# tataganesh/Query-Efficient-Approx-to-improve-OCR

Measured on AMD Instinct MI355X. Metric: patch-images/sec UNet->CRNN->CTC fwd+bwd, 32x128 grey, higher is better.
Workload: dtype f32 (GEMMs as scaled 2 x fp16 split products — three fp16 MFMAs per fp32 multiply-add — fp32 accumulate); 1 GPU; BASELINE configs[2]: full minibatch step of train_nn_area.py:212-287 — Phase A (UNet eval fwd, TopKCER k = 5 % of the minibatch, inner_limit = 4 jitter replicas fused in the batch dim, CRNN train-BN fwd+bwd, Adam(CRNN)) + Phase B (UNet train-BN -> CRNN BN-eval -> CTC mean + MSE -> backward -> Adam(UNet)) + greedy decode -> CER -> update_cer (:290-304) on synthetic POS-style 32x128 patches; batch_per_gpu=2048, global_batch=2048, full_step=True, crnn_wgrad=True, parallelism=dp1, hipgraph=False

## Files before the change

query-efficient-approx-to-improve-ocr_amd/csrc/conv_halo16.hip:

```cpp
#include "conv_args.h"
#include <type_traits>

using qea_conv::ConvArgs;

namespace {

__device__ const float qea_zero16[4] = {0.f, 0.f, 0.f, 0.f};

constexpr int halo_m16_wgs(int cout) { return cout == 32 ? 3 : 2; }

template <int COUT, bool STATS, int IMW = 0, int PKW = 0, bool BST = false>
__global__ __launch_bounds__(256) __attribute__((amdgpu_waves_per_eu(halo_m16_wgs(COUT), halo_m16_wgs(COUT)))) void conv3x3_halo_m16_kernel(
    const float* __restrict__ x, const _Float16* __restrict__ wf, float* __restrict__ y, int B, int H, int W, int ldx, int ldy,
    const float* __restrict__ scale, const float* __restrict__ bias, int relu, double* __restrict__ stats, int chunks, int Ntot,
    const float* __restrict__ mask, int ldmask, int total, const float* __restrict__ xmax, float* __restrict__ yamax, float* __restrict__ pooled,
    int ldp, float* __restrict__ pamax, const float* __restrict__ yref, int ldyref, const double* __restrict__ bst64, const float* __restrict__ bsc,
    const float* __restrict__ bsh) {
  constexpr int CIN = 64, TH = 4;
  constexpr bool SMALL = IMW != 0;
  constexpr int IMH = SMALL ? IMW / 4 : 1;
  constexpr int IPX = SMALL ? 32 / IMW : 1, IPY = SMALL ? TH / IMH : 1;
  constexpr int TW = 32, HW_ = SMALL ? IPX * (IMW + 2) : TW + 2, HH = SMALL ? TH + 1 : TH + 2, HP = HH * HW_;
  static_assert(!SMALL || COUT == 128, "small-image tiles: one wave row");
  constexpr int WN = COUT / 32, WM = 4 / WN, MI = TH / WM;
// ... 313 lines not shown
      }
      if (relu) {
#pragma unroll
        for (int i = 0; i < MI; ++i)
#pragma unroll
          for (int t = 0; t < 4; ++t)
#pragma unroll
            for (int r = 0; r < 4; ++r) acc[i][t][r] = fmaxf(acc[i][t][r], 0.f);
      }
      auto store_rows = [&](auto has_mask) {
        constexpr bool HAS_MASK = decltype(has_mask)::value;
#pragma unroll
        for (int i = 0; i < MI; ++i) {
          const int rowpix = (cur.b * H + cur.y0 + wm * MI + i) * W + cur.x0;
          float* yb = y + (size_t)rowpix * ldy;
          const float* mb = HAS_MASK ? mask + (size_t)rowpix * ldmask : nullptr;
          const int lo = 4 * lg * ldy + nbase, lom = 4 * lg * ldmask + nbase;
#pragma unroll
          for (int e = 0; e < 16; ++e) {
            const int g2 = (e >> 2) & 1;
            const int c = (e >> 3) * 16 + (e & 3);
            float v = acc[i][e >> 2][e & 3];
            if (SMALL) {
              const int px = c + 4 * lg;
              const int img = (i / IMH) * IPX + px / IMW;
              const size_t prow = ((size_t)(cur.b + img) * IMH + i % IMH) * IMW + px % IMW;
              if (cur.b + img >= B) continue;
              const int n = nbase + g2 * 16;
              if (HAS_MASK) v = (mask[prow * ldmask + n] > 0.f) ? v : 0.f;
              y[prow * ldy + n] = v;
            } else {
              if (HAS_MASK) v = (mb[lom + c * ldmask + g2 * 16] > 0.f) ? v : 0.f;
              yb[lo + c * ldy + g2 * 16] = v;
            }
            am = qea_amax_acc(am, v);
            if (STATS) {
              st0[g2] += (double)v;
              st1[g2] += (double)v * (double)v;
            }
          }
        }
      };
      if (mask) store_rows(std::true_type{});
      else store_rows(std::false_type{});
    }
    if (STATS || BST) {
#pragma unroll
      for (int g2 = 0; g2 < 2; ++g2) {
        double sa = st0[g2], sc = st1[g2];
        sa += __shfl_xor(sa, 16, 64);
        sc += __shfl_xor(sc, 16, 64);
        sa += __shfl_xor(sa, 32, 64);
        sc += __shfl_xor(sc, 32, 64);
        if (lg == 0) {
          double* dst = stats + ((size_t)(cur.tile_id * WM + wm) * Ntot + nbase + g2 * 16) * 2;
          dst[0] = sa;
          dst[1] = sc;
        }
      }
    }
    if (!has_next) break;
    cur = nxt;
    vb = nvb;
  }
  qea_amax_commit_block(am, yamax);
  if constexpr (PKW != 0) qea_amax_commit_block(pm, pamax);
}

template <int COUT, bool STATS, int IMW = 0, int PKW = 0, bool BST = false>
int launch_halo_m16_(const ConvArgs& a, hipStream_t s) {
  constexpr size_t lds = IMW ? (size_t)2 * (4 + 1) * (32 / IMW) * (IMW + 2) * 64 * 2 : (size_t)2 * (4 + 2) * 34 * 64 * 2;
  auto kern = conv3x3_halo_m16_kernel<COUT, STATS, IMW, PKW, BST>;
  static int attr_rc = (int)hipFuncSetAttribute((const void*)kern, hipFuncAttributeMaxDynamicSharedMemorySize, (int)lds);
  if (attr_rc != (int)hipSuccess) {
    qea_set_error("qea_conv_igemm(halo m16): cannot reserve %zu bytes of LDS: %s", (size_t)lds, hipGetErrorString((hipError_t)attr_rc));
    return QEA_ERR_LAUNCH;
  }
  const long long total = IMW ? (long long)qea_cdiv(a.B, (32 / IMW) * (4 / (IMW / 4))) * (a.N / COUT) : (long long)a.B * (a.H / 4) * (a.W / 32) * (a.N / COUT);
  if (total <= 0 || total > 0x7fffffffLL) {
    qea_set_error("qea_conv_igemm(halo m16): grid %lld out of range", total);
    return QEA_ERR_INVALID;
  }
  static const int resident = [] {
    int dev = 0, cus = 256;
    (void)hipGetDevice(&dev);
    (void)hipDeviceGetAttribute(&cus, hipDeviceAttributeMultiprocessorCount, dev);
    return halo_m16_wgs(COUT) * (cus & ~7);
  }();
  const unsigned grid = (total > resident && COUT > 32) ? (unsigned)resident : (unsigned)total;
  hipLaunchKernelGGL(kern, dim3(grid), dim3(256), lds, s, a.x, (const _Float16*)a.wp, a.y, a.B, a.H, a.W, a.ldx, a.ldy, a.scale, a.bias, a.relu, a.stats,
                     a.Cin / 64, a.N, a.mask, a.ldmask, (int)total, a.xmax, a.yamax, a.pool_y, a.ldpool, a.pool_amax, a.bst_y, a.ldbst, a.bst64, a.bst_scale,
                     a.bst_shift);
  return QEA_OK;
}

template <int COUT, int IMW = 0>
int launch_halo_m16(const ConvArgs& a, hipStream_t s) {
  if (a.pool_y) {
    if constexpr (COUT != 32 && IMW != 8) {
      if (a.pool_kw == 1) {
        if constexpr (COUT == 128 && IMW == 0) return launch_halo_m16_<COUT, false, IMW, 1>(a, s);
      } else {
        return launch_halo_m16_<COUT, false, IMW, 2>(a, s);
      }
    }
    qea_set_error("qea_conv_igemm(halo m16): no fused-pool instance for this shape");
    return QEA_ERR_INVALID;
  }
  if (a.bst_y) return launch_halo_m16_<COUT, false, IMW, 0, true>(a, s);
  return a.stats ? launch_halo_m16_<COUT, true, IMW>(a, s) : launch_halo_m16_<COUT, false, IMW>(a, s);
}

}

namespace qea_conv {

int launch_halo_m16_any(int n_sel, int sm, const ConvArgs& a, hipStream_t s) {
  if (sm == 16) return launch_halo_m16<128, 16>(a, s);
  if (sm == 8) return launch_halo_m16<128, 8>(a, s);
  if (n_sel == 32) return launch_halo_m16<32>(a, s);
  if (n_sel == 64) return launch_halo_m16<64>(a, s);
  return launch_halo_m16<128>(a, s);
}

}
```

query-efficient-approx-to-improve-ocr_amd/csrc/conv_igemm.hip:

```cpp
#include "conv_args.h"
#include <type_traits>
#include <stdlib.h>
#include <string.h>

using qea_conv::ConvArgs;
using qea_conv::conv_epilogue;

namespace {

template <int A_LD, int B_LD, int BK, int RPP>
struct IgemmGather {
  int lrow, kc, ntaps;
  int a_pix[A_LD];
  int a_ih0[A_LD], a_iw0[A_LD];
  const float* b_ptr[B_LD > 0 ? B_LD : 1];
  f32x4 a_reg[A_LD], b_reg[B_LD > 0 ? B_LD : 1];

  __device__ __forceinline__ void init(const ConvArgs& p, int tid, int m0, int n0) {
    constexpr int KCH = BK / 4;
    lrow = tid / KCH;
    kc = tid % KCH;
    ntaps = p.KH * p.KW;
    const int ohw = p.OH * p.OW;
#pragma unroll
// ... 1226 lines not shown
              st1 += (double)v * (double)v;
            }
          }
        }
      };
      if (mask) store_rows(std::true_type{});
      else store_rows(std::false_type{});
    }
    if (STATS || BST) {
      const double sa = st0 + __shfl_xor(st0, 32, 64);
      const double sc = st1 + __shfl_xor(st1, 32, 64);
      if (fh == 0) {
        double* dst = stats + ((size_t)(cur.tile_id * WM + wm) * Ntot + n) * 2;
        dst[0] = sa;
        dst[1] = sc;
      }
    }
    if (!has_next) break;
    cur = nxt;
    vb = nvb;
  }
  qea_amax_commit_block(am, yamax);
  if constexpr (PKW != 0) qea_amax_commit_block(pm, pamax);
}

__global__ void pack_frag_planes_kernel(const float* __restrict__ w, __bf16* __restrict__ dst, int N, int Cin, int CW) {
  const int NB = N > 128 ? 128 : N;
  const int KSr = CW / 16, WNr = NB / 32, chunks = Cin / CW;
  const int i = blockIdx.x * blockDim.x + threadIdx.x;
  if (i >= (N / NB) * chunks * 9 * KSr * WNr * 64) return;
  const int lane = i & 63;
  const int nj = (i >> 6) % WNr;
  const int gst = (i >> 6) / WNr;
  const int nbk = gst / (chunks * 9 * KSr);
  const int chunk = (gst / (9 * KSr)) % chunks, st = gst % (9 * KSr);
  const int tap = st / KSr, cs = st % KSr;
  const int n = nbk * NB + nj * 32 + (lane & 31);
  const float* src = w + ((size_t)n * 9 + tap) * Cin + chunk * CW + cs * 16 + 8 * (lane >> 5);
  const f32x4 v0 = *reinterpret_cast<const f32x4*>(src), v1 = *reinterpret_cast<const f32x4*>(src + 4);
  bf16x4 h0, m0, l0, h1, m1, l1;
  qea_split3(v0, h0, m0, l0);
  qea_split3(v1, h1, m1, l1);
  bf16x8 pl[3];
#pragma unroll
  for (int k = 0; k < 4; ++k) {
    pl[0][k] = h0[k]; pl[0][k + 4] = h1[k];
    pl[1][k] = m0[k]; pl[1][k + 4] = m1[k];
    pl[2][k] = l0[k]; pl[2][k + 4] = l1[k];
  }
#pragma unroll
  for (int p = 0; p < 3; ++p) *reinterpret_cast<bf16x8*>(dst + ((((size_t)gst * 3 + p) * WNr + nj) * 64 + lane) * 8) = pl[p];
}

__global__ void pack_frag_planes_f16_kernel(const float* __restrict__ w, _Float16* __restrict__ dst, int N, int Cin, int CW,
                                            const float* __restrict__ wmax) {
  const int NB = N > 128 ? 128 : N;
  const int KSr = CW / 16, WNr = NB / 32, chunks = Cin / CW;
  float sw, inv;
  qea_f16_scale(wmax[0], sw, inv);
  const int i = blockIdx.x * blockDim.x + threadIdx.x;
  if (i == 0) reinterpret_cast<float*>(dst + (size_t)N * 9 * Cin * 2)[0] = inv;
  if (i >= (N / NB) * chunks * 9 * KSr * WNr * 64) return;
  const int lane = i & 63;
  const int nj = (i >> 6) % WNr;
  const int gst = (i >> 6) / WNr;
  const int nbk = gst / (chunks * 9 * KSr);
  const int chunk = (gst / (9 * KSr)) % chunks, st = gst % (9 * KSr);
  const int tap = st / KSr, cs = st % KSr;
  const int n = nbk * NB + nj * 32 + (lane & 31);
  const float* src = w + ((size_t)n * 9 + tap) * Cin + chunk * CW + cs * 16 + 8 * (lane >> 5);
  const f32x4 v0 = *reinterpret_cast<const f32x4*>(src), v1 = *reinterpret_cast<const f32x4*>(src + 4);
  f16x4 h0, l0, h1, l1;
  qea_split2_f16(v0, sw, h0, l0);
  qea_split2_f16(v1, sw, h1, l1);
  f16x8 pl[2];
#pragma unroll
  for (int k = 0; k < 4; ++k) {
    pl[0][k] = h0[k]; pl[0][k + 4] = h1[k];
    pl[1][k] = l0[k]; pl[1][k + 4] = l1[k];
  }
#pragma unroll
  for (int p = 0; p < 2; ++p) *reinterpret_cast<f16x8*>(dst + ((((size_t)gst * 2 + p) * WNr + nj) * 64 + lane) * 8) = pl[p];
}

__global__ void pack_frag_planes_f16_m16_kernel(const float* __restrict__ w, _Float16* __restrict__ dst, int N, int Cin, const float* __restrict__ wmax) {
  const int NB = N > 128 ? 128 : N;
  const int NGr = NB / 16, chunks = Cin / 64;
  float sw, inv;
  qea_f16_scale(wmax[0], sw, inv);
  const int i = blockIdx.x * blockDim.x + threadIdx.x;
  if (i == 0) reinterpret_cast<float*>(dst + (size_t)N * 9 * Cin * 2)[0] = inv;
  if (i >= (N / NB) * chunks * 18 * NGr * 64) return;
  const int lane = i & 63;
  const int ng = (i >> 6) % NGr;
  const int gst = (i >> 6) / NGr;
  const int nbk = gst / (chunks * 18);
  const int chunk = (gst / 18) % chunks, st = gst % 18;
  const int tap = st / 2, ks = st % 2;
  const int n = nbk * NB + ng * 16 + (lane & 15);
  const float* src = w + ((size_t)n * 9 + tap) * Cin + chunk * 64 + ks * 32 + 8 * (lane >> 4);
  const f32x4 v0 = *reinterpret_cast<const f32x4*>(src), v1 = *reinterpret_cast<const f32x4*>(src + 4);
  f16x4 h0, l0, h1, l1;
  qea_split2_f16(v0, sw, h0, l0);
  qea_split2_f16(v1, sw, h1, l1);
  f16x8 pl[2];
#pragma unroll
  for (int k = 0; k < 4; ++k) {
    pl[0][k] = h0[k]; pl[0][k + 4] = h1[k];
    pl[1][k] = l0[k]; pl[1][k + 4] = l1[k];
  }
#pragma unroll
  for (int p = 0; p < 2; ++p) *reinterpret_cast<f16x8*>(dst + ((((size_t)gst * 2 + p) * NGr + ng) * 64 + lane) * 8) = pl[p];
}

template <int CIN, int COUT, int TH, bool STATS, int IMW = 0, int NPL = 3, int PKW = 0, bool BST = false>
int launch_halo_bf3_(const ConvArgs& a, hipStream_t s) {
  constexpr size_t lds = IMW ? (size_t)NPL * (TH + 1) * (32 / IMW) * (IMW + 2) * CIN * 2 : (size_t)NPL * (TH + 2) * 34 * CIN * 2;
  auto kern = conv3x3_halo_bf3_kernel<CIN, COUT, TH, STATS, IMW, NPL, PKW, BST>;
  static int attr_rc = (int)hipFuncSetAttribute((const void*)kern, hipFuncAttributeMaxDynamicSharedMemorySize, (int)lds);
  if (attr_rc != (int)hipSuccess) {
    qea_set_error("qea_conv_igemm(halo bf3): cannot reserve %zu bytes of LDS: %s", (size_t)lds, hipGetErrorString((hipError_t)attr_rc));
    return QEA_ERR_LAUNCH;
  }
  const long long total = IMW ? (long long)qea_cdiv(a.B, (32 / IMW) * (TH / (IMW / 4))) * (a.N / COUT)
                              : (long long)a.B * (a.H / TH) * (a.W / 32) * (a.N / COUT);
  if (total <= 0 || total > 0x7fffffffLL) {
    qea_set_error("qea_conv_igemm(halo bf3): grid %lld out of range", total);
    return QEA_ERR_INVALID;
  }
  static const int resident = [] {
    int dev = 0, cus = 256;
    (void)hipGetDevice(&dev);
    (void)hipDeviceGetAttribute(&cus, hipDeviceAttributeMultiprocessorCount, dev);
    return halo_bf3_wgs(CIN, COUT, NPL, BST) * (cus & ~7);
  }();
  const unsigned grid = (total > resident && COUT > 32) ? (unsigned)resident : (unsigned)total;
  hipLaunchKernelGGL(kern, dim3(grid), dim3(256), lds, s, a.x, (const __bf16*)a.wp, a.y, a.B, a.H, a.W, a.ldx, a.ldy,
                     a.scale, a.bias, a.relu, a.stats, a.Cin / CIN, a.N, a.mask, a.ldmask, (int)total, a.xmax, a.yamax, a.pool_y, a.ldpool, a.pool_amax,
                     a.bst_y, a.ldbst, a.bst64, a.bst_scale, a.bst_shift);
  return QEA_OK;
}

template <int CIN, int COUT, int TH, int IMW = 0>
int launch_halo_bf3_pool(const ConvArgs& a, hipStream_t s) {
  if (a.pool_kw == 1) return launch_halo_bf3_<CIN, COUT, TH, false, IMW, 2, 1>(a, s);
  return launch_halo_bf3_<CIN, COUT, TH, false, IMW, 2, 2>(a, s);
}

template <int CIN, int COUT, int TH, int IMW = 0>
int launch_halo_bf3(const ConvArgs& a, hipStream_t s) {
  if (a.xmax && a.bst_y)
    return launch_halo_bf3_<CIN, COUT, TH, false, IMW, 2, 0, true>(a, s);
  if (a.xmax)
    return a.stats ? launch_halo_bf3_<CIN, COUT, TH, true, IMW, 2>(a, s) : launch_halo_bf3_<CIN, COUT, TH, false, IMW, 2>(a, s);
  return a.stats ? launch_halo_bf3_<CIN, COUT, TH, true, IMW>(a, s) : launch_halo_bf3_<CIN, COUT, TH, false, IMW>(a, s);
}

bool halo_eligible(const qea_conv_desc* d) {
  const bool ch = (d->Cin == 32 || d->Cin == 64) && (d->N == 32 || d->N == 64);
  const int th = d->Cin == 32 ? 8 : 4;
  return ch && d->KH == 3 && d->KW == 3 && d->pad_h == 1 && d->pad_w == 1 && d->stride_h == 1 && d->stride_w == 1 && d->OH == d->H &&
         d->OW == d->W && d->W % 32 == 0 && d->H % th == 0 && d->out_mode == QEA_OUT_NHWC && !d->mask && !d->accumulate;
}

int halo_bf3_small(const qea_conv_desc* d) {
  if (d->Cin % 64 || d->Cin > 512 || d->N % 128) return 0;
  if (d->W == 16 && d->H == 4) return 16;
  if (d->W == 8 && d->H == 2) return 8;
  return 0;
}

bool halo_bf3_eligible(const qea_conv_desc* d) {
  const bool cin = d->Cin == 32 || (d->Cin % 64 == 0 && d->Cin <= 512);
  const bool cout = d->N == 32 || d->N == 64 || d->N % 128 == 0;
  const int th = d->Cin == 32 ? 8 : 4;
  const bool shape = (d->W % 32 == 0 && d->H % th == 0) || halo_bf3_small(d) != 0;
  return cin && cout && d->KH == 3 && d->KW == 3 && d->pad_h == 1 && d->pad_w == 1 && d->stride_h == 1 && d->stride_w == 1 && d->OH == d->H &&
         d->OW == d->W && shape && d->out_mode == QEA_OUT_NHWC && !d->accumulate;
}

long long halo_bf3_tiles(const qea_conv_desc* d) {
  const int sm = halo_bf3_small(d);
  if (sm) return qea_cdiv(d->B, (32 / sm) * (4 / (sm / 4)));
  return (long long)d->B * (d->H / (d->Cin == 32 ? 8 : 4)) * (d->W / 32);
}

bool halo_bf3_pool_shape(const qea_conv_desc* d, int kw) {
  if (!halo_bf3_eligible(d) || d->mask || d->stats || d->H % 2 || (kw != 1 && kw != 2) || (kw == 2 && d->W % 2)) return false;
  const int sm = halo_bf3_small(d);
  if (sm == 16) return kw == 2;
  if (sm) return false;
  if (d->Cin == 32) return d->N == 32 && kw == 2;
  if (d->N == 64) return kw == 2;
  return d->N % 128 == 0;
}

int launch_halo_bf3_any(const qea_conv_desc* d, const ConvArgs& a, hipStream_t s) {
  const int sm = halo_bf3_small(d);
  if (a.xmax && d->Cin % 64 == 0) {
    return qea_conv::launch_halo_m16_any(d->N == 32 ? 32 : (d->N == 64 ? 64 : 128), sm, a, s);
  }
  if (a.pool_y) {
    if (sm == 16) return launch_halo_bf3_<64, 128, 4, false, 16, 2, 2>(a, s);
    if (d->Cin == 32) return launch_halo_bf3_<32, 32, 8, false, 0, 2, 2>(a, s);
    if (d->N == 64) return launch_halo_bf3_<64, 64, 4, false, 0, 2, 2>(a, s);
    return launch_halo_bf3_pool<64, 128, 4>(a, s);
  }
  if (sm == 16) return launch_halo_bf3<64, 128, 4, 16>(a, s);
  if (sm == 8) return launch_halo_bf3<64, 128, 4, 8>(a, s);
  if (d->Cin == 32) {
    if (d->N == 32) return launch_halo_bf3<32, 32, 8>(a, s);
    if (d->N == 64) return launch_halo_bf3<32, 64, 8>(a, s);
    return launch_halo_bf3<32, 128, 8>(a, s);
  }
  if (d->N == 32) return launch_halo_bf3<64, 32, 4>(a, s);
  if (d->N == 64) return launch_halo_bf3<64, 64, 4>(a, s);
  return launch_halo_bf3<64, 128, 4>(a, s);
}

int halo_bf3_wm(const qea_conv_desc* d) { return 4 / ((d->N > 128 ? 128 : d->N) / 32); }

int launch_halo_any(const qea_conv_desc* d, const ConvArgs& a, hipStream_t s) {
  if (d->Cin == 32 && d->N == 32) return launch_halo<32, 32, 8>(a, s);
  if (d->Cin == 32 && d->N == 64) return launch_halo<32, 64, 8>(a, s);
  if (d->Cin == 64 && d->N == 32) return launch_halo<64, 32, 4>(a, s);
  return launch_halo<64, 64, 4>(a, s);
}

bool halo_bf3_wins(const qea_conv_desc* d) { return halo_bf3_eligible(d); }

bool gemm1x1_eligible(const qea_conv_desc* d) {
  return d->KH == 1 && d->KW == 1 && d->stride_h == 1 && d->stride_w == 1 && d->pad_h == 0 && d->pad_w == 0 && d->OH == d->H && d->OW == d->W &&
         d->Cin % 64 == 0 && d->N % 128 == 0 && !d->scale && !d->mask && !d->accumulate && !d->stats &&
         (long long)d->N * d->Cin * 4 < 0x7fffffffLL &&
         (d->out_mode != QEA_OUT_CONVT || (long long)d->B * d->H * d->W * 4 < 0x7fffffffLL);
}

int pick_tile(const qea_conv_desc* d, const ConvArgs& a) {
  int tile = 0;
  const long long tiles128 = (long long)qea_cdiv(a.M, 128) * qea_cdiv(d->N, 128);
  const long long tiles7 = (long long)qea_cdiv(a.M, 256) * qea_cdiv(d->N, 128);
  const long long tiles8 = (long long)qea_cdiv(a.M, 128) * qea_cdiv(d->N, 256);
  const long long tiles21 = (long long)qea_cdiv(a.M, 256) * qea_cdiv(d->N, 128);
  const long long tiles22 = (long long)qea_cdiv(a.M, 128) * qea_cdiv(d->N, 256);
  const bool bf3 = qea_split_bf16_enabled() && d->N >= 128 && a.K >= 256;
  if (qea_split_bf16_enabled() && d->tile != -1 && gemm1x1_eligible(d)) tile = 26;
  else if (qea_split_bf16_enabled() && d->tile != -1 && halo_bf3_wins(d)) tile = 24;
  else if (qea_split_bf16_enabled() && d->N > 32 && d->N <= 64 && a.K >= 256 && d->Cin >= 64) tile = 23;
  else if (halo_eligible(d)) tile = 4;
  else if (qea_split_bf16_enabled() && (d->out_mode == QEA_OUT_CONVT || (d->stride_h == 2 && d->stride_w == 2)) && d->N >= 64 && a.K >= 64 &&
           a.K <= 256 && d->Cin % 16 == 0)
    tile = 25;
  else if (d->N <= 32) tile = 3;
  else if (d->N <= 64) tile = 9;
  else if (bf3 && d->N % 256 == 0 && tiles22 >= 512) tile = 22;
  else if (bf3 && tiles21 >= 512) tile = 21;
  else if (bf3) tile = 25;
  else if (d->N % 256 == 0 && tiles8 >= 1024) tile = 8;
  else if (tiles7 >= 512) tile = 7;
// ... 186 lines not shown
  if (!d || d->Cin <= 0 || d->Cin % 32 || d->B <= 0) return 0;
  ConvArgs a;
  memset(&a, 0, sizeof(a));
  a.M = d->B * d->OH * d->OW;
  a.N = d->N;
  a.K = d->KH * d->KW * d->Cin;
  const int tile = d->tile ? d->tile : pick_tile(d, a);
  return tile >= 20 ? 1 : 0;
}

extern "C" size_t qea_split_planes_bytes(int64_t M, int32_t C) { return (size_t)M * (size_t)C * 6 + 128; }

extern "C" int qea_split_planes(const float* x, int32_t ld, int64_t M, int32_t C, void* planes, void* stream) {
  QEA_REQUIRE(x && planes && M > 0 && C > 0 && C % 16 == 0 && ld >= C && ld % 4 == 0, "qea_split_planes: bad arguments (C=%d must be a multiple of 16)", C);
  QEA_REQUIRE(((uintptr_t)x & 15) == 0 && ((uintptr_t)planes & 15) == 0, "qea_split_planes: pointers must be 16-byte aligned");
  const long long total = M * (C >> 3);
  const long long blocks = (total + 255) / 256;
  QEA_REQUIRE(blocks < 0x7fffffffLL, "qea_split_planes: too large");
  hipLaunchKernelGGL(split_planes_kernel, dim3((unsigned)blocks), dim3(256), 0, (hipStream_t)stream, x, ld, (long long)M, C, (__bf16*)planes);
  QEA_CHECK_LAUNCH();
  return QEA_OK;
}

extern "C" size_t qea_split_planes_f16_bytes(int64_t M, int32_t C) { return (size_t)M * (size_t)C * 4 + 128 + 16; }

extern "C" int qea_split_planes_f16(const float* x, int32_t ld, int64_t M, int32_t C, const float* xmax, void* planes, void* stream) {
  QEA_REQUIRE(x && planes && xmax && M > 0 && C > 0 && C % 16 == 0 && ld >= C && ld % 4 == 0, "qea_split_planes_f16: bad arguments (C=%d must be a multiple of 16)", C);
  QEA_REQUIRE(((uintptr_t)x & 15) == 0 && ((uintptr_t)planes & 15) == 0, "qea_split_planes_f16: pointers must be 16-byte aligned");
  const long long total = M * (C >> 3);
  const long long blocks = (total + 255) / 256;
  QEA_REQUIRE(blocks < 0x7fffffffLL, "qea_split_planes_f16: too large");
  hipLaunchKernelGGL(split_planes_f16_kernel, dim3((unsigned)blocks), dim3(256), 0, (hipStream_t)stream, x, ld, (long long)M, C, xmax, (_Float16*)planes);
  QEA_CHECK_LAUNCH();
  return QEA_OK;
}

extern "C" size_t qea_pack_frag_planes_bytes(int32_t N, int32_t Cin) { return (size_t)N * 9 * Cin * 6; }

extern "C" int qea_pack_frag_planes(const float* w, int32_t N, int32_t Cin, void* planes, void* stream) {
  QEA_REQUIRE(w && planes && (N == 32 || N == 64 || (N > 0 && N % 128 == 0)) && (Cin == 32 || (Cin % 64 == 0 && Cin <= 512)),
              "qea_pack_frag_planes: N in {32, 64, 128k}, Cin = 32 or a multiple of 64 up to 512");
  const int total = 9 * (Cin / 16) * (N / 32) * 64;
  hipLaunchKernelGGL(pack_frag_planes_kernel, dim3(qea_cdiv(total, 256)), dim3(256), 0, (hipStream_t)stream, w, (__bf16*)planes, N, Cin,
                     Cin == 32 ? 32 : 64);
  QEA_CHECK_LAUNCH();
  return QEA_OK;
}

extern "C" size_t qea_pack_frag_planes_f16_bytes(int32_t N, int32_t Cin) { return (size_t)N * 9 * Cin * 4 + 16; }

extern "C" int qea_pack_frag_planes_f16(const float* w, int32_t N, int32_t Cin, const float* wmax, void* planes, void* stream) {
  QEA_REQUIRE(w && planes && wmax && (N == 32 || N == 64 || (N > 0 && N % 128 == 0)) && (Cin == 32 || (Cin % 64 == 0 && Cin <= 512)),
              "qea_pack_frag_planes_f16: N in {32, 64, 128k}, Cin = 32 or a multiple of 64 up to 512");
  if (Cin % 64 == 0) {
    const int total16 = 9 * (Cin / 32) * (N / 16) * 64;
    hipLaunchKernelGGL(pack_frag_planes_f16_m16_kernel, dim3(qea_cdiv(total16, 256)), dim3(256), 0, (hipStream_t)stream, w, (_Float16*)planes, N, Cin, wmax);
    QEA_CHECK_LAUNCH();
    return QEA_OK;
  }
  const int total = 9 * (Cin / 16) * (N / 32) * 64;
  hipLaunchKernelGGL(pack_frag_planes_f16_kernel, dim3(qea_cdiv(total, 256)), dim3(256), 0, (hipStream_t)stream, w, (_Float16*)planes, N, Cin,
                     Cin == 32 ? 32 : 64, wmax);
  QEA_CHECK_LAUNCH();
  return QEA_OK;
}

extern "C" int qea_conv_igemm_wants_frag_planes(const qea_conv_desc* d) {
  if (!d || d->Cin <= 0 || d->Cin % 32 || d->B <= 0) return 0;
  ConvArgs a;
  memset(&a, 0, sizeof(a));
  a.M = d->B * d->OH * d->OW;
  a.N = d->N;
  a.K = d->KH * d->KW * d->Cin;
  const int tile = d->tile ? d->tile : pick_tile(d, a);
  return tile == 24 ? 1 : (tile == 26 ? 2 : 0);
}
```

query-efficient-approx-to-improve-ocr_amd/csrc/weight_forms.hip:

```cpp
#include "common.h"
#include "../../include/qea_hip.h"

namespace {

constexpr int MAXJ = 64;
struct JobTable {
  qea_wform_job j[MAXJ];
};

__device__ __forceinline__ void split_store2(const float* src, float sw, _Float16* d0, _Float16* d1) {
  const f32x4 v0 = *reinterpret_cast<const f32x4*>(src), v1 = *reinterpret_cast<const f32x4*>(src + 4);
  f16x4 h0, l0, h1, l1;
  qea_split2_f16(v0, sw, h0, l0);
  qea_split2_f16(v1, sw, h1, l1);
  f16x8 ph, pl;
#pragma unroll
  for (int k = 0; k < 4; ++k) {
    ph[k] = h0[k]; ph[k + 4] = h1[k];
    pl[k] = l0[k]; pl[k + 4] = l1[k];
  }
  *reinterpret_cast<f16x8*>(d0) = ph;
  *reinterpret_cast<f16x8*>(d1) = pl;
}

__global__ __launch_bounds__(256) void weight_forms_multi_kernel(const JobTable t) {
  const qea_wform_job& jb = t.j[blockIdx.y];
  const float* w = jb.src;
  const long long stride = (long long)gridDim.x * 256;
  const long long i0 = (long long)blockIdx.x * 256 + threadIdx.x;
  if (jb.kind == 0) {
    const int Co = jb.a, Ci = jb.b, KH = jb.c, KW = jb.d;
    float* wt = (float*)jb.dst;
    const long long n = (long long)Co * KH * KW * Ci;
    for (long long i = i0; i < n; i += stride) {
      const int co = (int)(i % Co);
      long long r = i / Co;
      const int kw2 = (int)(r % KW);
      r /= KW;
      const int kh2 = (int)(r % KH);
      const int ci = (int)(r / KH);
      wt[i] = w[(((size_t)co * KH + (KH - 1 - kh2)) * KW + (KW - 1 - kw2)) * Ci + ci];
    }
    return;
  }
  float sw, inv;
  qea_f16_scale(jb.amax[0], sw, inv);
  _Float16* dst = (_Float16*)jb.dst;
  if (jb.kind == 1) {
    const int N = jb.a, Cin = jb.b;
    const int NB = N > 128 ? 128 : N;
    if (i0 == 0) reinterpret_cast<float*>(dst + (size_t)N * 9 * Cin * 2)[0] = inv;
    if (Cin % 64 == 0) {
      const int NGr = NB / 16, chunks = Cin / 64;
      const long long total = (long long)(N / NB) * chunks * 18 * NGr * 64;
      for (long long ii = i0; ii < total; ii += stride) {
        const int i = (int)ii, lane = i & 63;
        const int ng = (i >> 6) % NGr;
        const int gst = (i >> 6) / NGr;
        const int nbk = gst / (chunks * 18);
        const int chunk = (gst / 18) % chunks, st = gst % 18;
        const int tap = st / 2, ks = st % 2;
        const int n = nbk * NB + ng * 16 + (lane & 15);
        const float* src = w + ((size_t)n * 9 + tap) * Cin + chunk * 64 + ks * 32 + 8 * (lane >> 4);
        _Float16* o = dst + ((((size_t)gst * 2) * NGr + ng) * 64 + lane) * 8;
        split_store2(src, sw, o, o + (size_t)NGr * 64 * 8);
      }
    } else {
      const int CW = Cin == 32 ? 32 : 64;
      const int KSr = CW / 16, WNr = NB / 32, chunks = Cin / CW;
      const long long total = (long long)(N / NB) * chunks * 9 * KSr * WNr * 64;
      for (long long ii = i0; ii < total; ii += stride) {
        const int i = (int)ii, lane = i & 63;
        const int nj = (i >> 6) % WNr;
        const int gst = (i >> 6) / WNr;
        const int nbk = gst / (chunks * 9 * KSr);
        const int chunk = (gst / (9 * KSr)) % chunks, st = gst % (9 * KSr);
        const int tap = st / KSr, cs = st % KSr;
        const int n = nbk * NB + nj * 32 + (lane & 31);
        const float* src = w + ((size_t)n * 9 + tap) * Cin + chunk * CW + cs * 16 + 8 * (lane >> 5);
        _Float16* o = dst + ((((size_t)gst * 2) * WNr + nj) * 64 + lane) * 8;
        split_store2(src, sw, o, o + (size_t)WNr * 64 * 8);
      }
    }
    return;
  }
  const int N = jb.a, K = jb.b, chunks = K / 64;
  if (i0 == 0) reinterpret_cast<float*>(dst + (size_t)N * K * 2)[0] = inv;
  const long long total = (long long)(N / 128) * chunks * 4 * 4 * 64;
  for (long long ii = i0; ii < total; ii += stride) {
    const int i = (int)ii, lane = i & 63;
    const int nj = (i >> 6) & 3;
    const int gst = i >> 8;
    const int nbk = gst / (chunks * 4);
    const int chunk = (gst >> 2) % chunks, cs = gst & 3;
    const int n = nbk * 128 + nj * 32 + (lane & 31);
    const float* src = w + (size_t)n * K + chunk * 64 + cs * 16 + 8 * (lane >> 5);
    _Float16* o = dst + ((((size_t)gst * 2) * 4 + nj) * 64 + lane) * 8;
    split_store2(src, sw, o, o + (size_t)4 * 64 * 8);
  }
}

}

extern "C" int qea_weight_forms_multi(const qea_wform_job* jobs, int32_t n, void* stream) {
  QEA_REQUIRE(jobs && n > 0 && n <= MAXJ, "qea_weight_forms_multi: 1 to 64 jobs");
  JobTable t;
  long long most = 0;
  for (int i = 0; i < n; ++i) {
    const qea_wform_job& j = jobs[i];
    QEA_REQUIRE(j.src && j.dst && j.kind >= 0 && j.kind <= 2 && (j.kind == 0 || j.amax), "qea_weight_forms_multi: null pointer or unknown kind in a job");
    QEA_REQUIRE(((uintptr_t)j.src & 15) == 0 && ((uintptr_t)j.dst & 15) == 0, "qea_weight_forms_multi: pointers must be 16-byte aligned");
    long long items;
    if (j.kind == 0) {
      QEA_REQUIRE(j.a > 0 && j.b > 0 && j.c > 0 && j.d > 0, "qea_weight_forms_multi: bad flip-transpose shape");
      items = (long long)j.a * j.b * j.c * j.d;
    } else if (j.kind == 1) {
      QEA_REQUIRE((j.a == 32 || j.a == 64 || (j.a > 0 && j.a % 128 == 0)) && (j.b == 32 || (j.b % 64 == 0 && j.b > 0 && j.b <= 512)),
                  "qea_weight_forms_multi: 3x3 planes need N in {32, 64, 128k}, Cin = 32 or a multiple of 64 up to 512");
      items = j.b % 64 == 0 ? 9LL * (j.b / 32) * (j.a / 16) * 64 : 9LL * (j.b / 16) * (j.a / 32) * 64;
    } else {
      QEA_REQUIRE(j.a > 0 && j.a % 128 == 0 && j.b > 0 && j.b % 64 == 0 && (long long)j.a * j.b * 4 < 0x7fffffffLL,
                  "qea_weight_forms_multi: 1x1 planes need N a multiple of 128, K a multiple of 64");
      items = (long long)(j.a / 128) * (j.b / 64) * 4 * 4 * 64;
    }
    QEA_REQUIRE(items < 0x7fffffffLL, "qea_weight_forms_multi: a job is too large");
    if (items > most) most = items;
    t.j[i] = j;
  }
  long long gx = (most + 255) / 256;
  if (gx > 512) gx = 512;
  hipLaunchKernelGGL(weight_forms_multi_kernel, dim3((unsigned)gx, (unsigned)n), dim3(256), 0, (hipStream_t)stream, t);
  QEA_CHECK_LAUNCH();
  return QEA_OK;
}
```

Measured before the change: 22720 patch-images/s.

## Add 16x16x32 fp16 halo conv kernel for 32-input-channel layers

Adds a dedicated halo-tiled 3x3 conv kernel for Cin=32 that uses 16x16x32 fp16 MFMAs with 8-row tiles, covering the plain, stats, fused-pool and BatchNorm-backward epilogues. It routes all fp16-split convs through the m16 path and drops the older 32x32 bf16 packing and kernel variants for Cin=32. Weight packing now emits only the m16 fragment layout. The stats store indexing is also corrected to per-lane channels. The goal is to remove the slower 32x32-fragment path for the shallow UNet layers, in exchange for new code with its own register and occupancy tuning.

```diff
diff --git a/query-efficient-approx-to-improve-ocr_amd/csrc/conv_halo16.hip b/query-efficient-approx-to-improve-ocr_amd/csrc/conv_halo16.hip
--- a/query-efficient-approx-to-improve-ocr_amd/csrc/conv_halo16.hip
+++ b/query-efficient-approx-to-improve-ocr_amd/csrc/conv_halo16.hip
@@ -389,8 +389,8 @@
         sc += __shfl_xor(sc, 16, 64);
         sa += __shfl_xor(sa, 32, 64);
         sc += __shfl_xor(sc, 32, 64);
-        if (lg == 0) {
-          double* dst = stats + ((size_t)(cur.tile_id * WM + wm) * Ntot + nbase + g2 * 16) * 2;
+        if (g4 == 0) {
+          double* dst = stats + ((size_t)(cur.tile_id * WM + wm) * Ntot + cur.nb * COUT + wn * 32 + p16 + g2 * 16) * 2;
           dst[0] = sa;
           dst[1] = sc;
         }
@@ -448,11 +448,405 @@
   return a.stats ? launch_halo_m16_<COUT, true, IMW>(a, s) : launch_halo_m16_<COUT, false, IMW>(a, s);
 }
 
+constexpr int halo_c32_wgs(int cout, bool bst) { return (cout == 64 || (cout == 128 && bst)) ? 2 : 3; }
+
+template <int COUT, bool STATS, int PKW = 0, bool BST = false>
+__global__ __launch_bounds__(256) __attribute__((amdgpu_waves_per_eu(halo_c32_wgs(COUT, BST), halo_c32_wgs(COUT, BST)))) void conv3x3_halo_m16_c32_kernel(
+    const float* __restrict__ x, const _Float16* __restrict__ wf, float* __restrict__ y, int B, int H, int W, int ldx, int ldy,
+    const float* __restrict__ scale, const float* __restrict__ bias, int relu, double* __restrict__ stats, int Ntot,
+    const float* __restrict__ mask, int ldmask, int total, const float* __restrict__ xmax, float* __restrict__ yamax, float* __restrict__ pooled,
+    int ldp, float* __restrict__ pamax, const float* __restrict__ yref, int ldyref, const double* __restrict__ bst64, const float* __restrict__ bsc,
+    const float* __restrict__ bsh) {
+  constexpr int CIN = 32, TH = 8, TW = 32, HW_ = TW + 2, HH = TH + 2, HP = HH * HW_;
+  constexpr int WN = COUT / 32, WM = 4 / WN, MI = TH / WM;
+  constexpr int MP = COUT == 128 ? 2 : MI;
+  constexpr int NG = COUT / 16;
+  constexpr int PLANE = HP * CIN, PLANE_B = PLANE * 2;
+  static_assert(MI % MP == 0 && MP % 2 == 0, "row passes: whole row pairs");
+  static_assert(PKW == 0 || (!STATS && (PKW == 1 || PKW == 2)), "fused pooling: no statistics");
+  static_assert(!BST || (!STATS && PKW == 0), "BatchNorm-backward sums: their own instances");
+  extern __shared__ __attribute__((aligned(16))) float smem[];
+  _Float16* As = reinterpret_cast<_Float16*>(smem);
+  float sx, inv_x;
+  qea_f16_scale(xmax[0], sx, inv_x);
+  const float inv_w = reinterpret_cast<const float*>(wf + (size_t)Ntot * 9 * CIN * 2)[0];
+
+  const int tiles_x = W / TW, tiles_y = H / TH;
+  const int nblk = Ntot / COUT;
+  struct Item { int nb, tile_id, b, x0, y0; };
+  auto decode = [&](int vb) {
+    const int lid = qea_xcd_swizzle(vb, total);
+    Item it;
+    it.nb = lid % nblk;
+    it.tile_id = lid / nblk;
+    int bid = it.tile_id;
+    const int tx = bid % tiles_x;
+    bid /= tiles_x;
+    const int ty = bid % tiles_y;
+    it.b = bid / tiles_y;
+    it.x0 = tx * TW;
+    it.y0 = ty * TH;
+    it.nb = __builtin_amdgcn_readfirstlane(it.nb);
+    it.tile_id = __builtin_amdgcn_readfirstlane(it.tile_id);
+    it.b = __builtin_amdgcn_readfirstlane(it.b);
+    it.x0 = __builtin_amdgcn_readfirstlane(it.x0);
+    it.y0 = __builtin_amdgcn_readfirstlane(it.y0);
+    return it;
+  };
+
+  constexpr int C4 = CIN / 4, NLD = (HP * C4 + 255) / 256, QS = 256 / C4;
+  f32x4 hv[NLD];
+  auto gather = [&](const Item& it, int tid) {
+    const float* xb = x + (size_t)it.b * H * W * ldx + (tid % C4) * 4;
+    int q = tid / C4;
+    int hy = 0, hx = q;
+#pragma unroll
+    for (int i = 0; i < NLD; ++i) {
+      const int iy = it.y0 + hy - 1, ix = it.x0 + hx - 1;
+      const bool ok = q < HP && (unsigned)iy < (unsigned)H && (unsigned)ix < (unsigned)W;
+      typedef const __attribute__((address_space(1))) f32x4* gptr;
+      const gptr pz = (gptr)(const void*)qea_zero16;
+      const gptr pv = (gptr)(const void*)(xb + ((size_t)iy * W + ix) * ldx);
+      hv[i] = *(ok ? pv : pz);
+      q += QS;
+      hx += QS;
+      if (hx >= HW_) {
+        hx -= HW_;
+        ++hy;
+      }
+    }
+  };
+  auto stage = [&](int tid) {
+    const int c4 = tid % C4;
+    int q = tid / C4;
+#pragma unroll
+    for (int i = 0; i < NLD; ++i) {
+      if (q < HP) {
+        const int o = q * CIN + (((c4 >> 1) ^ ((q >> 1) & 2)) << 3) + (c4 & 1) * 4;
+        f16x4 h, l;
+        qea_split2_f16(hv[i], sx, h, l);
+        *reinterpret_cast<f16x4*>(As + o) = h;
+        *reinterpret_cast<f16x4*>(As + PLANE + o) = l;
+      }
+      q += QS;
+    }
+  };
+
+  const int lane_ = threadIdx.x & 63, wave_ = threadIdx.x >> 6;
+  const int p16 = lane_ & 15, g4 = lane_ >> 4;
+  const int wm = wave_ / WN, wn = wave_ % WN;
+  int T[8];
+  auto table = [&](int ps) {
+    const int W0 = (wm * MI + ps * MP) * HW_;
+#pragma unroll
+    for (int k = 0; k < 8; ++k) {
+      const int p = W0 + p16 + k;
+      T[k] = p * (CIN * 2) + ((g4 ^ ((p >> 1) & 2)) << 4);
+    }
+  };
+  if (MI == MP) table(0);
+
+  f16x8 bq[2][2][2];
+  auto load_b = [&](int nb, int tap, int buf, int tid) {
+    const f16x8* wu = reinterpret_cast<const f16x8*>(wf) + (size_t)nb * 9 * 2 * NG * 64 + (size_t)tap * 2 * NG * 64;
+    const unsigned lo = (unsigned)(((tid >> 6) % WN) * 2) * 64 + (tid & 63);
+#pragma unroll
+    for (int pl = 0; pl < 2; ++pl)
+#pragma unroll
+      for (int g2 = 0; g2 < 2; ++g2) bq[buf][g2][pl] = (wu + (pl * NG + g2) * 64)[lo];
+  };
+
+  int vb = blockIdx.x;
+  Item cur = decode(vb);
+  gather(cur, threadIdx.x);
+  load_b(cur.nb, 0, 0, threadIdx.x);
+  bool first = true;
+  float am = 0.f, pm = 0.f;
+  while (true) {
+    const int nvb = vb + gridDim.x;
+    const bool has_next = nvb < total;
+    const Item nxt = decode(has_next ? nvb : vb);
+    int tid = threadIdx.x;
+    asm volatile("" : "+v"(tid));
+    if (!first) __syncthreads();
+    first = false;
+    stage(tid);
+    __syncthreads();
+    if (has_next) gather(nxt, tid);
+
+    double st0[2] = {0.0, 0.0}, st1[2] = {0.0, 0.0};
+
+#pragma unroll 1
+    for (int ps = 0; ps < MI / MP; ++ps) {
+      const bool last_pass = ps + 1 == MI / MP;
+      if (MI != MP) {
+        table(ps);
+        asm volatile("" : "+v"(tid));
+      }
+      f32x4 acc[MP][4];
+#pragma unroll
+      for (int i = 0; i < MP; ++i)
+#pragma unroll
+        for (int t = 0; t < 4; ++t)
+#pragma unroll
+          for (int r = 0; r < 4; ++r) acc[i][t][r] = 0.f;
+      constexpr int GR = MP * 2;
+      auto read_a = [&](int tap, int g, f16x8* a) {
+        const int kh = tap / 3, kw = tap % 3;
+        const int i = g / 2, xh = g % 2;
+        const int c = (i + kh) * HW_ + kw + xh * 16;
+        const char* src = reinterpret_cast<const char*>(As) + T[c & 7] + (c >> 3) * 512;
+        a[0] = *reinterpret_cast<const f16x8*>(src);
+        a[1] = *reinterpret_cast<const f16x8*>(src + PLANE_B);
+      };
+      f16x8 ar[2][2];
+      read_a(0, 0, ar[0]);
+#pragma unroll
+      for (int st = 0; st < 9; ++st) {
+        const int cb = st & 1;
+        if (st + 1 < 9) load_b(cur.nb, st + 1, cb ^ 1, tid);
+        __builtin_amdgcn_sched_barrier(0);
+#pragma unroll
+        for (int g = 0; g < GR; ++g) {
+          const int f = st * GR + g;
+          const f16x8* a = ar[f & 1];
+          const bool more = f + 1 < 9 * GR;
+          if (more) read_a((f + 1) / GR, (f + 1) % GR, ar[(f + 1) & 1]);
+          const int i = g / 2, xh = g % 2;
+#pragma unroll
+          for (int g2 = 0; g2 < 2; ++g2) acc[i][xh * 2 + g2] = __builtin_amdgcn_mfma_f32_16x16x32_f16(a[1], bq[cb][g2][0], acc[i][xh * 2 + g2], 0, 0, 0);
+#pragma unroll
+          for (int g2 = 0; g2 < 2; ++g2) acc[i][xh * 2 + g2] = __builtin_amdgcn_mfma_f32_16x16x32_f16(a[0], bq[cb][g2][1], acc[i][xh * 2 + g2], 0, 0, 0);
+#pragma unroll
+          for (int g2 = 0; g2 < 2; ++g2) acc[i][xh * 2 + g2] = __builtin_amdgcn_mfma_f32_16x16x32_f16(a[0], bq[cb][g2][0], acc[i][xh * 2 + g2], 0, 0, 0);
+          if (more) {
+            __builtin_amdgcn_sched_group_barrier(0x100, 2, 0);
+            __builtin_amdgcn_sched_group_barrier(0x008, 6, 0);
+          }
+        }
+      }
+
+      if (!last_pass) load_b(cur.nb, 0, 0, tid);
+      else if (has_next) load_b(nxt.nb, 0, 0, tid);
+
+      __builtin_amdgcn_sched_barrier(0);
+      int etid = threadIdx.x;
+      asm volatile("" : "+v"(etid));
+      const int lp = etid & 15, lg = (etid & 63) >> 4;
+      const int nbase = cur.nb * COUT + (((etid >> 6) % WN) * 32) + lp;
+      float esc[2], ebi[2];
+#pragma unroll
+      for (int g2 = 0; g2 < 2; ++g2) {
+        esc[g2] = scale ? scale[nbase + g2 * 16] : 1.f;
+        ebi[g2] = bias ? bias[nbase + g2 * 16] : 0.f;
+      }
+      auto e_px = [&](int e) { return (e >> 3) * 16 + 4 * lg + (e & 3); };
+      const int row0 = cur.y0 + wm * MI + ps * MP;
+      if constexpr (PKW != 0) {
+#pragma unroll
+        for (int i = 0; i < MP; i += 2) {
+          float vv[2][16];
+#pragma unroll
+          for (int ii = 0; ii < 2; ++ii)
+#pragma unroll
+            for (int e = 0; e < 16; ++e) {
+              const int g2 = (e >> 2) & 1, n = nbase + g2 * 16;
+              const size_t prow = (size_t)(cur.b * H + row0 + i + ii) * W + cur.x0 + e_px(e);
+              float v = (acc[i + ii][e >> 2][e & 3] * inv_x) * inv_w;
+              if (scale && bias) v = __fmaf_rn(v, esc[g2], ebi[g2]);
+              else if (scale) v *= esc[g2];
+              else if (bias) v += ebi[g2];
+              if (relu) v = fmaxf(v, 0.f);
+              vv[ii][e] = v;
+              y[prow * ldy + n] = v;
+              am = qea_amax_acc(am, v);
+            }
+#pragma unroll
+          for (int e = 0; e < 16; e += PKW) {
+            const int g2 = (e >> 2) & 1, n = nbase + g2 * 16;
+            const int px = e_px(e);
+            float m = -INFINITY;
+#pragma unroll
+            for (int ii = 0; ii < 2; ++ii)
+#pragma unroll
+              for (int jj = 0; jj < PKW; ++jj) {
+                const float v = vv[ii][e + jj];
+                m = (v > m || v != v) ? v : m;
+              }
+            const size_t prow = ((size_t)cur.b * (H / 2) + (row0 + i) / 2) * (W / PKW) + (cur.x0 + px) / PKW;
+            pooled[prow * ldp + n] = m;
+            pm = qea_amax_acc(pm, m);
+          }
+        }
+      } else if constexpr (BST) {
+        float msc[2], msh[2];
+        double bmu[2], bis[2];
+#pragma unroll
+        for (int g2 = 0; g2 < 2; ++g2) {
+          msc[g2] = bsc[nbase + g2 * 16];
+          msh[g2] = bsh[nbase + g2 * 16];
+          bmu[g2] = bst64[nbase + g2 * 16];
+          bis[g2] = bst64[Ntot + nbase + g2 * 16];
+        }
+#pragma unroll
+        for (int i = 0; i < MP; ++i) {
+          const size_t rowpix = (size_t)(cur.b * H + row0 + i) * W + cur.x0;
+          float* yb = y + rowpix * ldy;
+          const float* rb = yref + rowpix * ldyref;
+          const float* mb = mask ? mask + rowpix * ldmask : nullptr;
+          const unsigned lo = 4 * lg * ldy + nbase, lor = 4 * lg * ldyref + nbase, lom = 4 * lg * ldmask + nbase;
+#pragma unroll
+          for (int e = 0; e < 16; ++e) {
+            const int g2 = (e >> 2) & 1;
+            const int c = (e >> 3) * 16 + (e & 3);
+            float v = (acc[i][e >> 2][e & 3] * inv_x) * inv_w;
+            if (scale && bias) v = __fmaf_rn(v, esc[g2], ebi[g2]);
+            else if (scale) v *= esc[g2];
+            else if (bias) v += ebi[g2];
+            if (relu) v = fmaxf(v, 0.f);
+            if (mask) v = ((mb + (c * ldmask + g2 * 16))[lom] > 0.f) ? v : 0.f;
+            (yb + (c * ldy + g2 * 16))[lo] = v;
+            am = qea_amax_acc(am, v);
+            const float yv = (rb + (c * ldyref + g2 * 16))[lor];
+            const float dz = __fmaf_rn(yv, msc[g2], msh[g2]) > 0.f ? v : 0.f;
+            st0[g2] += (double)dz;
+            st1[g2] += (double)dz * (((double)yv - bmu[g2]) * bis[g2]);
+          }
+          __builtin_amdgcn_sched_barrier(0);
+        }
+      } else {
+#pragma unroll
+        for (int i = 0; i < MP; ++i)
+#pragma unroll
+          for (int t = 0; t < 4; ++t)
+#pragma unroll
+            for (int r = 0; r < 4; ++r) acc[i][t][r] = (acc[i][t][r] * inv_x) * inv_w;
+        if (scale && bias) {
+#pragma unroll
+          for (int i = 0; i < MP; ++i)
+#pragma unroll
+            for (int t = 0; t < 4; ++t)
+#pragma unroll
+              for (int r = 0; r < 4; ++r) acc[i][t][r] = __fmaf_rn(acc[i][t][r], esc[t & 1], ebi[t & 1]);
+        } else if (scale) {
+#pragma unroll
+          for (int i = 0; i < MP; ++i)
+#pragma unroll
+            for (int t = 0; t < 4; ++t)
+#pragma unroll
+              for (int r = 0; r < 4; ++r) acc[i][t][r] *= esc[t & 1];
+        } else if (bias) {
+#pragma unroll
+          for (int i = 0; i < MP; ++i)
+#pragma unroll
+            for (int t = 0; t < 4; ++t)
+#pragma unroll
+              for (int r = 0; r < 4; ++r) acc[i][t][r] += ebi[t & 1];
+        }
+        if (relu) {
+#pragma unroll
+          for (int i = 0; i < MP; ++i)
+#pragma unroll
+            for (int t = 0; t < 4; ++t)
+#pragma unroll
+              for (int r = 0; r < 4; ++r) acc[i][t][r] = fmaxf(acc[i][t][r], 0.f);
+        }
+        auto store_rows = [&](auto has_mask) {
+          constexpr bool HAS_MASK = decltype(has_mask)::value;
+#pragma unroll
+          for (int i = 0; i < MP; ++i) {
+            const size_t rowpix = (size_t)(cur.b * H + row0 + i) * W + cur.x0;
+            float* yb = y + rowpix * ldy;
+            const float* mb = HAS_MASK ? mask + rowpix * ldmask : nullptr;
+            const unsigned lo = 4 * lg * ldy + nbase, lom = 4 * lg * ldmask + nbase;
+#pragma unroll
+            for (int e = 0; e < 16; ++e) {
+              const int g2 = (e >> 2) & 1;
+              const int c = (e >> 3) * 16 + (e & 3);
+              float v = acc[i][e >> 2][e & 3];
+              if (HAS_MASK) v = ((mb + (c * ldmask + g2 * 16))[lom] > 0.f) ? v : 0.f;
+              (yb + (c * ldy + g2 * 16))[lo] = v;
+              am = qea_amax_acc(am, v);
+              if (STATS) {
+                st0[g2] += (double)v;
+                st1[g2] += (double)v * (double)v;
+              }
+            }
+          }
+        };
+        if (mask) store_rows(std::true_type{});
+        else store_rows(std::false_type{});
+      }
+      __builtin_amdgcn_sched_barrier(0);
+    }
+    if (STATS || BST) {
+#pragma unroll
+      for (int g2 = 0; g2 < 2; ++g2) {
+        double sa = st0[g2], sc = st1[g2];
+        sa += __shfl_xor(sa, 16, 64);
+        sc += __shfl_xor(sc, 16, 64);
+        sa += __shfl_xor(sa, 32, 64);
+        sc += __shfl_xor(sc, 32, 64);
+        if (g4 == 0) {
+          double* dst = stats + ((size_t)(cur.tile_id * WM + wm) * Ntot + cur.nb * COUT + wn * 32 + p16 + g2 * 16) * 2;
+          dst[0] = sa;
+          dst[1] = sc;
+        }
+      }
+    }
+    if (!has_next) break;
+    cur = nxt;
+    vb = nvb;
+  }
+  qea_amax_commit_block(am, yamax);
+  if constexpr (PKW != 0) qea_amax_commit_block(pm, pamax);
 }
 
+template <int COUT, bool STATS, int PKW = 0, bool BST = false>
+int launch_halo_c32_(const ConvArgs& a, hipStream_t s) {
+  constexpr size_t lds = (size_t)2 * (8 + 2) * 34 * 32 * 2;
+  auto kern = conv3x3_halo_m16_c32_kernel<COUT, STATS, PKW, BST>;
+  const long long total = (long long)a.B * (a.H / 8) * (a.W / 32) * (a.N / COUT);
+  if (total <= 0 || total > 0x7fffffffLL) {
+    qea_set_error("qea_conv_igemm(halo m16, 32 channels): grid %lld out of range", total);
+    return QEA_ERR_INVALID;
+  }
+  static const int resident = [] {
+    int dev = 0, cus = 256;
+    (void)hipGetDevice(&dev);
+    (void)hipDeviceGetAttribute(&cus, hipDeviceAttributeMultiprocessorCount, dev);
+    return halo_c32_wgs(COUT, BST) * (cus & ~7);
+  }();
+  const unsigned grid = total > resident ? (unsigned)resident : (unsigned)total;
+  hipLaunchKernelGGL(kern, dim3(grid), dim3(256), lds, s, a.x, (const _Float16*)a.wp, a.y, a.B, a.H, a.W, a.ldx, a.ldy, a.scale, a.bias, a.relu, a.stats,
+                     a.N, a.mask, a.ldmask, (int)total, a.xmax, a.yamax, a.pool_y, a.ldpool, a.pool_amax, a.bst_y, a.ldbst, a.bst64, a.bst_scale,
+                     a.bst_shift);
+  return QEA_OK;
+}
+
+template <int COUT>
+int launch_halo_c32(const ConvArgs& a, hipStream_t s) {
+  if (a.pool_y) {
+    if constexpr (COUT == 32) {
+      if (a.pool_kw == 2) return launch_halo_c32_<COUT, false, 2>(a, s);
+    }
+    qea_set_error("qea_conv_igemm(halo m16, 32 channels): no fused-pool instance for this shape");
+    return QEA_ERR_INVALID;
+  }
+  if (a.bst_y) return launch_halo_c32_<COUT, false, 0, true>(a, s);
+  return a.stats ? launch_halo_c32_<COUT, true>(a, s) : launch_halo_c32_<COUT, false>(a, s);
+}
+
+}
+
 namespace qea_conv {
 
 int launch_halo_m16_any(int n_sel, int sm, const ConvArgs& a, hipStream_t s) {
+  if (a.Cin == 32) {
+    if (n_sel == 32) return launch_halo_c32<32>(a, s);
+    if (n_sel == 64) return launch_halo_c32<64>(a, s);
+    return launch_halo_c32<128>(a, s);
+  }
   if (sm == 16) return launch_halo_m16<128, 16>(a, s);
   if (sm == 8) return launch_halo_m16<128, 8>(a, s);
   if (n_sel == 32) return launch_halo_m16<32>(a, s);
diff --git a/query-efficient-approx-to-improve-ocr_amd/csrc/conv_igemm.hip b/query-efficient-approx-to-improve-ocr_amd/csrc/conv_igemm.hip
--- a/query-efficient-approx-to-improve-ocr_amd/csrc/conv_igemm.hip
+++ b/query-efficient-approx-to-improve-ocr_amd/csrc/conv_igemm.hip
@@ -1302,53 +1302,23 @@
   for (int p = 0; p < 3; ++p) *reinterpret_cast<bf16x8*>(dst + ((((size_t)gst * 3 + p) * WNr + nj) * 64 + lane) * 8) = pl[p];
 }
 
-__global__ void pack_frag_planes_f16_kernel(const float* __restrict__ w, _Float16* __restrict__ dst, int N, int Cin, int CW,
-                                            const float* __restrict__ wmax) {
+__global__ void pack_frag_planes_f16_m16_kernel(const float* __restrict__ w, _Float16* __restrict__ dst, int N, int Cin, const float* __restrict__ wmax) {
   const int NB = N > 128 ? 128 : N;
-  const int KSr = CW / 16, WNr = NB / 32, chunks = Cin / CW;
+  const int CW = Cin == 32 ? 32 : 64, KSr = CW / 32, SPC = 9 * KSr;
+  const int NGr = NB / 16, chunks = Cin / CW;
   float sw, inv;
   qea_f16_scale(wmax[0], sw, inv);
   const int i = blockIdx.x * blockDim.x + threadIdx.x;
   if (i == 0) reinterpret_cast<float*>(dst + (size_t)N * 9 * Cin * 2)[0] = inv;
-  if (i >= (N / NB) * chunks * 9 * KSr * WNr * 64) return;
-  const int lane = i & 63;
-  const int nj = (i >> 6) % WNr;
-  const int gst = (i >> 6) / WNr;
-  const int nbk = gst / (chunks * 9 * KSr);
-  const int chunk = (gst / (9 * KSr)) % chunks, st = gst % (9 * KSr);
-  const int tap = st / KSr, cs = st % KSr;
-  const int n = nbk * NB + nj * 32 + (lane & 31);
-  const float* src = w + ((size_t)n * 9 + tap) * Cin + chunk * CW + cs * 16 + 8 * (lane >> 5);
-  const f32x4 v0 = *reinterpret_cast<const f32x4*>(src), v1 = *reinterpret_cast<const f32x4*>(src + 4);
-  f16x4 h0, l0, h1, l1;
-  qea_split2_f16(v0, sw, h0, l0);
-  qea_split2_f16(v1, sw, h1, l1);
-  f16x8 pl[2];
-#pragma unroll
-  for (int k = 0; k < 4; ++k) {
-    pl[0][k] = h0[k]; pl[0][k + 4] = h1[k];
-    pl[1][k] = l0[k]; pl[1][k + 4] = l1[k];
-  }
-#pragma unroll
-  for (int p = 0; p < 2; ++p) *reinterpret_cast<f16x8*>(dst + ((((size_t)gst * 2 + p) * WNr + nj) * 64 + lane) * 8) = pl[p];
-}
-
-__global__ void pack_frag_planes_f16_m16_kernel(const float* __restrict__ w, _Float16* __restrict__ dst, int N, int Cin, const float* __restrict__ wmax) {
-  const int NB = N > 128 ? 128 : N;
-  const int NGr = NB / 16, chunks = Cin / 64;
-  float sw, inv;
-  qea_f16_scale(wmax[0], sw, inv);
-  const int i = blockIdx.x * blockDim.x + threadIdx.x;
-  if (i == 0) reinterpret_cast<float*>(dst + (size_t)N * 9 * Cin * 2)[0] = inv;
-  if (i >= (N / NB) * chunks * 18 * NGr * 64) return;
+  if (i >= (N / NB) * chunks * SPC * NGr * 64) return;
   const int lane = i & 63;
   const int ng = (i >> 6) % NGr;
   const int gst = (i >> 6) / NGr;
-  const int nbk = gst / (chunks * 18);
-  const int chunk = (gst / 18) % chunks, st = gst % 18;
-  const int tap = st / 2, ks = st % 2;
+  const int nbk = gst / (chunks * SPC);
+  const int chunk = (gst / SPC) % chunks, st = gst % SPC;
+  const int tap = st / KSr, ks = st % KSr;
   const int n = nbk * NB + ng * 16 + (lane & 15);
-  const float* src = w + ((size_t)n * 9 + tap) * Cin + chunk * 64 + ks * 32 + 8 * (lane >> 4);
+  const float* src = w + ((size_t)n * 9 + tap) * Cin + chunk * CW + ks * 32 + 8 * (lane >> 4);
   const f32x4 v0 = *reinterpret_cast<const f32x4*>(src), v1 = *reinterpret_cast<const f32x4*>(src + 4);
   f16x4 h0, l0, h1, l1;
   qea_split2_f16(v0, sw, h0, l0);
@@ -1392,17 +1362,7 @@
 }
 
 template <int CIN, int COUT, int TH, int IMW = 0>
-int launch_halo_bf3_pool(const ConvArgs& a, hipStream_t s) {
-  if (a.pool_kw == 1) return launch_halo_bf3_<CIN, COUT, TH, false, IMW, 2, 1>(a, s);
-  return launch_halo_bf3_<CIN, COUT, TH, false, IMW, 2, 2>(a, s);
-}
-
-template <int CIN, int COUT, int TH, int IMW = 0>
 int launch_halo_bf3(const ConvArgs& a, hipStream_t s) {
-  if (a.xmax && a.bst_y)
-    return launch_halo_bf3_<CIN, COUT, TH, false, IMW, 2, 0, true>(a, s);
-  if (a.xmax)
-    return a.stats ? launch_halo_bf3_<CIN, COUT, TH, true, IMW, 2>(a, s) : launch_halo_bf3_<CIN, COUT, TH, false, IMW, 2>(a, s);
   return a.stats ? launch_halo_bf3_<CIN, COUT, TH, true, IMW>(a, s) : launch_halo_bf3_<CIN, COUT, TH, false, IMW>(a, s);
 }
 
@@ -1447,14 +1407,12 @@
 
 int launch_halo_bf3_any(const qea_conv_desc* d, const ConvArgs& a, hipStream_t s) {
   const int sm = halo_bf3_small(d);
-  if (a.xmax && d->Cin % 64 == 0) {
+  if (a.xmax) {
     return qea_conv::launch_halo_m16_any(d->N == 32 ? 32 : (d->N == 64 ? 64 : 128), sm, a, s);
   }
-  if (a.pool_y) {
-    if (sm == 16) return launch_halo_bf3_<64, 128, 4, false, 16, 2, 2>(a, s);
-    if (d->Cin == 32) return launch_halo_bf3_<32, 32, 8, false, 0, 2, 2>(a, s);
-    if (d->N == 64) return launch_halo_bf3_<64, 64, 4, false, 0, 2, 2>(a, s);
-    return launch_halo_bf3_pool<64, 128, 4>(a, s);
+  if (a.pool_y || a.bst_y) {
+    qea_set_error("qea_conv_igemm(halo bf3): the fused pool and the BatchNorm-backward sums need the fp16 operands");
+    return QEA_ERR_INVALID;
   }
   if (sm == 16) return launch_halo_bf3<64, 128, 4, 16>(a, s);
   if (sm == 8) return launch_halo_bf3<64, 128, 4, 8>(a, s);
@@ -1747,15 +1705,8 @@
 extern "C" int qea_pack_frag_planes_f16(const float* w, int32_t N, int32_t Cin, const float* wmax, void* planes, void* stream) {
   QEA_REQUIRE(w && planes && wmax && (N == 32 || N == 64 || (N > 0 && N % 128 == 0)) && (Cin == 32 || (Cin % 64 == 0 && Cin <= 512)),
               "qea_pack_frag_planes_f16: N in {32, 64, 128k}, Cin = 32 or a multiple of 64 up to 512");
-  if (Cin % 64 == 0) {
-    const int total16 = 9 * (Cin / 32) * (N / 16) * 64;
-    hipLaunchKernelGGL(pack_frag_planes_f16_m16_kernel, dim3(qea_cdiv(total16, 256)), dim3(256), 0, (hipStream_t)stream, w, (_Float16*)planes, N, Cin, wmax);
-    QEA_CHECK_LAUNCH();
-    return QEA_OK;
-  }
-  const int total = 9 * (Cin / 16) * (N / 32) * 64;
-  hipLaunchKernelGGL(pack_frag_planes_f16_kernel, dim3(qea_cdiv(total, 256)), dim3(256), 0, (hipStream_t)stream, w, (_Float16*)planes, N, Cin,
-                     Cin == 32 ? 32 : 64, wmax);
+  const int total16 = 9 * (Cin / 32) * (N / 16) * 64;
+  hipLaunchKernelGGL(pack_frag_planes_f16_m16_kernel, dim3(qea_cdiv(total16, 256)), dim3(256), 0, (hipStream_t)stream, w, (_Float16*)planes, N, Cin, wmax);
   QEA_CHECK_LAUNCH();
   return QEA_OK;
 }
diff --git a/query-efficient-approx-to-improve-ocr_amd/csrc/weight_forms.hip b/query-efficient-approx-to-improve-ocr_amd/csrc/weight_forms.hip
--- a/query-efficient-approx-to-improve-ocr_amd/csrc/weight_forms.hip
+++ b/query-efficient-approx-to-improve-ocr_amd/csrc/weight_forms.hip
@@ -50,36 +50,21 @@
     const int N = jb.a, Cin = jb.b;
     const int NB = N > 128 ? 128 : N;
     if (i0 == 0) reinterpret_cast<float*>(dst + (size_t)N * 9 * Cin * 2)[0] = inv;
-    if (Cin % 64 == 0) {
-      const int NGr = NB / 16, chunks = Cin / 64;
-      const long long total = (long long)(N / NB) * chunks * 18 * NGr * 64;
+    {
+      const int CW = Cin == 32 ? 32 : 64, KSr = CW / 32, SPC = 9 * KSr;
+      const int NGr = NB / 16, chunks = Cin / CW;
+      const long long total = (long long)(N / NB) * chunks * SPC * NGr * 64;
       for (long long ii = i0; ii < total; ii += stride) {
         const int i = (int)ii, lane = i & 63;
         const int ng = (i >> 6) % NGr;
         const int gst = (i >> 6) / NGr;
-        const int nbk = gst / (chunks * 18);
-        const int chunk = (gst / 18) % chunks, st = gst % 18;
-        const int tap = st / 2, ks = st % 2;
+        const int nbk = gst / (chunks * SPC);
+        const int chunk = (gst / SPC) % chunks, st = gst % SPC;
+        const int tap = st / KSr, ks = st % KSr;
         const int n = nbk * NB + ng * 16 + (lane & 15);
-        const float* src = w + ((size_t)n * 9 + tap) * Cin + chunk * 64 + ks * 32 + 8 * (lane >> 4);
+        const float* src = w + ((size_t)n * 9 + tap) * Cin + chunk * CW + ks * 32 + 8 * (lane >> 4);
         _Float16* o = dst + ((((size_t)gst * 2) * NGr + ng) * 64 + lane) * 8;
         split_store2(src, sw, o, o + (size_t)NGr * 64 * 8);
-      }
-    } else {
-      const int CW = Cin == 32 ? 32 : 64;
-      const int KSr = CW / 16, WNr = NB / 32, chunks = Cin / CW;
-      const long long total = (long long)(N / NB) * chunks * 9 * KSr * WNr * 64;
-      for (long long ii = i0; ii < total; ii += stride) {
-        const int i = (int)ii, lane = i & 63;
-        const int nj = (i >> 6) % WNr;
-        const int gst = (i >> 6) / WNr;
-        const int nbk = gst / (chunks * 9 * KSr);
-        const int chunk = (gst / (9 * KSr)) % chunks, st = gst % (9 * KSr);
-        const int tap = st / KSr, cs = st % KSr;
-        const int n = nbk * NB + nj * 32 + (lane & 31);
-        const float* src = w + ((size_t)n * 9 + tap) * Cin + chunk * CW + cs * 16 + 8 * (lane >> 5);
-        _Float16* o = dst + ((((size_t)gst * 2) * WNr + nj) * 64 + lane) * 8;
-        split_store2(src, sw, o, o + (size_t)WNr * 64 * 8);
       }
     }
     return;
@@ -117,7 +102,7 @@
     } else if (j.kind == 1) {
       QEA_REQUIRE((j.a == 32 || j.a == 64 || (j.a > 0 && j.a % 128 == 0)) && (j.b == 32 || (j.b % 64 == 0 && j.b > 0 && j.b <= 512)),
                   "qea_weight_forms_multi: 3x3 planes need N in {32, 64, 128k}, Cin = 32 or a multiple of 64 up to 512");
-      items = j.b % 64 == 0 ? 9LL * (j.b / 32) * (j.a / 16) * 64 : 9LL * (j.b / 16) * (j.a / 32) * 64;
+      items = 9LL * (j.b / 32) * (j.a / 16) * 64;
     } else {
       QEA_REQUIRE(j.a > 0 && j.a % 128 == 0 && j.b > 0 && j.b % 64 == 0 && (long long)j.a * j.b * 4 < 0x7fffffffLL,
                   "qea_weight_forms_multi: 1x1 planes need N a multiple of 128, K a multiple of 64");
```

Result: no change. 22720 patch-images/s (median of 2 runs) (+0.0%).
